# wesselb/stheno

Measured on AMD Instinct MI355X. Metric: GP logpdf+posterior evals/sec at N=16384 D=8 fp64, higher is better.
Workload: dtype f64; 1 GPU; EQ() kernel, N=16384 D=8 fp64, logpdf + condition, posterior mean/var at N*=2048; nan_scan=every step (the library's per-tensor memo is cleared at the start of each step), call_order=posterior-first, info_check=behind the call that factorised (the library's default), parallelism=replicas only (1 independent evals in flight, one process per GPU)

## Files before the change

stheno_amd/csrc/gpk_potrf.hip:

```cpp
#include "gpk_common.hpp"
#include "gpk_gemm_tile.hpp"
#include "gpk_potrf_pipe.hpp"
#include <vector>

namespace {

constexpr int LDP = 130;

template <typename T>
struct DiagArgs {
    T* A;
    int64_t ld, bstride, off;
    int n;
    T* dinv;
    int64_t dinv_bstride;
    int* info;
    int info_base;
    long long* prof;
    int zero_next;
    T* rhs = nullptr;
    int64_t rhs_stride = 0;
};

#define PROF_MARK(i)                                                            \
// ... 1074 lines not shown

void gpk_set_diag_prof(long long* dev_buf) { g_diag_prof = dev_buf; }

GPK_KNOB(int, g_batch_mixed, 1);
GPK_KNOB(int64_t, g_batch_mixed_min, 64);
GPK_KNOB(int, g_batch_lag, 96);

static bool stream_has_all_cus(hipStream_t stream) {
    if (stream == nullptr) return true;
    int dev = 0, cus = 0;
    if (hipGetDevice(&dev) != hipSuccess || hipDeviceGetAttribute(&cus, hipDeviceAttributeMultiprocessorCount, dev) != hipSuccess || cus < 1 ||
        cus > 32 * 32)
        return false;
    const uint32_t words = (uint32_t)((cus + 31) / 32);
    uint32_t mask[32];
    for (uint32_t i = 0; i < 32; ++i) mask[i] = 0u;
    if (hipExtStreamGetCUMask(stream, words, mask) != hipSuccess) {
        (void)hipGetLastError();
        return false;
    }
    int set = 0;
    for (uint32_t i = 0; i < words; ++i) set += __builtin_popcount(mask[i]);
    return set >= cus;
}

template <typename T>
struct RhsRide {
    T* B;
    int64_t sB;
    T* tmp;
    bool done;
};
template <typename T>
static int potrf_batched_mixed(T* A, int64_t n, int64_t ld, int64_t batch, int64_t bstride, T* dinv, int64_t dstride, int* info, int nbo,
                               int info_base, hipStream_t stream, RhsRide<T>* ride = nullptr) {
    const int nblk = (int)(n / GPK_DB), npb = nbo / GPK_DB;
    for (int jn = 0; jn < nblk; ++jn) {
        const bool below = jn + 1 < nblk;
        DiagArgs<T> d;
        d.A = A; d.ld = ld; d.bstride = bstride; d.off = (int64_t)jn * GPK_DB; d.n = (int)n;
        d.dinv = dinv; d.dinv_bstride = dstride; d.info = info; d.info_base = info_base;
        d.prof = g_diag_prof;
        d.zero_next = below ? 1 : 0;
        if (ride != nullptr) { d.rhs = ride->B; d.rhs_stride = ride->sB; }
        launch_diag<T>(d, (unsigned)batch, stream);
        GPK_CHECK_LAUNCH();
        if (!below) break;
        BatchStepArgs<T> p;
        p.rhs = ride != nullptr ? ride->B : nullptr;
        p.srhs = ride != nullptr ? ride->sB : 0;
        p.A = A; p.ld = ld; p.bstride = bstride; p.n = (int)n; p.batch = (int)batch;
        p.dinv = dinv; p.dstride = dstride; p.info = info;
        p.jn = jn;
        p.tm = nblk - jn - 1;
        const int jl = jn % npb;
        if (jl == npb - 1) {
            p.K = nbo; p.tn = p.tm;
        } else {
            int z = 0;
            while ((jl >> z) & 1) ++z;
            p.K = GPK_DB << z;
            p.tn = (p.K / GPK_DB < p.tm) ? p.K / GPK_DB : p.tm;
        }
        p.nU = p.tm;
        for (int ti = 1; ti < p.tm; ++ti) p.nU += (ti < p.tn - 1) ? ti : p.tn - 1;
        p.lag = (g_batch_lag + p.tm + p.nU - 1) / (p.tm + p.nU);
        const int per_xcd = (int)((batch + 7) / 8);
        if (p.lag > per_xcd) p.lag = per_xcd;
        if (p.lag < 1) p.lag = 1;
        const int64_t qlen = (int64_t)(per_xcd + p.lag) * (p.tm + p.nU);
        const int ndiag = p.tn < p.tm ? p.tn : p.tm;
        const double fl = (double)batch * ((double)p.tm * GPK_DB * GPK_DB * GPK_DB + (2.0 * (p.nU - ndiag) + ndiag) * GPK_DB * GPK_DB * (double)p.K);
        void* slot = gpk_prof_begin(160 + (sizeof(T) == 8 ? 8 : 0), fl, stream);
        hipLaunchKernelGGL((batch_mix_kernel<T>), dim3((unsigned)(8 * qlen)), dim3(256), 0, stream, p);
        gpk_prof_end(slot, stream);
        GPK_CHECK_LAUNCH();
    }
    if (ride != nullptr) ride->done = true;
    return GPK_OK;
}

template <typename T>
static int potrf_plain(T* A, int64_t n, int64_t ld, int64_t batch, int64_t bstride, T* dinv,
                       int* info, int nbo, int info_base, hipStream_t stream, int64_t rows = 0, RhsRide<T>* rhs_ride = nullptr) {
    if (n <= 0 || batch <= 0) return GPK_OK;
    if (rows < n) rows = n;
    if (rows > INT32_MAX) return GPK_ERR_ARG(2);
    if (ld < n) return GPK_ERR_ARG(3);
    if (rows > n && (batch != 1 || dinv == nullptr || !g_pipe)) return GPK_ERR_ARG(2);
    if (nbo <= 0) nbo = (batch == 1 && dinv != nullptr) ? (n <= 4096 ? 4096 : (int)g_plain_nbo) : ((n >= 8192) ? 1024 : (n >= 2048 ? 512 : 256));
    if (nbo < GPK_DB || (nbo & (nbo - 1))) return GPK_ERR_ARG(9);
    if (info == nullptr) return GPK_ERR_ARG(7);
    if (dinv == nullptr && n > GPK_DB) return GPK_ERR_ARG(6);
    const int64_t nblk = gpk_cdiv(n, GPK_DB);
    const int64_t dstride = nblk * GPK_DB * GPK_DB;

    if constexpr (sizeof(T) == 4) {
        if (g_batch_mixed && batch >= g_batch_mixed_min && rows == n && dinv != nullptr && n % GPK_DB == 0 && n >= 4 * GPK_DB && nbo <= n &&
            n <= 64 * 1024 && stream_has_all_cus(stream) && ld % Traits<T>::VEC == 0 && bstride % Traits<T>::VEC == 0 && (uintptr_t)A % 16 == 0 &&
            (uintptr_t)dinv % 16 == 0 && ld < GPK_PIPE_LD_MAX && batch <= INT32_MAX / 8)
            return potrf_batched_mixed<T>(A, n, ld, batch, bstride, dinv, dstride, info, nbo, info_base, stream, rhs_ride);
    }

    PanelCtx<T> ctx{A, n, ld, batch, bstride, dinv, dstride, info, stream, info_base};
    ctx.rows = rows;
    const bool ride = g_pipe && g_pipe_fill && batch == 1 && dinv != nullptr;
    int64_t owed = 0;
    for (int64_t k0 = 0; k0 < n; k0 += nbo) {
        const int64_t k1 = (k0 + nbo < n) ? k0 + nbo : n;
        bool done = false;
        if (owed > 0) {
            const T* P = A + k0 * ld + (k0 - owed);
            int st = gpk_gemm_launch<T>(true, true, rows - k0, k1 - k0, owed, T(-1), P, ld, bstride, P, ld, bstride, T(1), A + k0 * ld + k0, ld,
                                        bstride, batch, true, stream);
            if (st) return st;
            if (k1 < n && n - k0 > GPK_DB) {
                st = potrf_panel_pipe<T>(ctx, k0, nbo, &done, owed);
                if (st) return st;
            }
            if (!done && k1 < n) {
                const T* P2 = A + k1 * ld + (k0 - owed);
                st = gpk_gemm_launch<T>(true, true, rows - k1, n - k1, owed, T(-1), P2, ld, bstride, P2, ld, bstride, T(1), A + k1 * ld + k1, ld,
                                        bstride, batch, true, stream);
                if (st) return st;
            }
            owed = 0;
        }
        if (!done) {
            int pst = potrf_panel_any<T>(ctx, k0, nbo);
            if (pst) return pst;
        }
        if (k1 < n) {
            if (ride && n - k1 > GPK_DB) {
                owed = k1 - k0;
            } else {
                const T* P = A + k1 * ld + k0;
                int st = gpk_gemm_launch<T>(true, true, rows - k1, n - k1, k1 - k0, T(-1), P, ld, bstride, P, ld,
                                            bstride, T(1), A + k1 * ld + k1, ld, bstride, batch, true, stream);
                if (st) return st;
            }
        }
    }
    return GPK_OK;
}


#include <mutex>

namespace {

struct LaDevice {
    hipStream_t aux = nullptr;
    hipStream_t priv = nullptr;
    std::vector<hipEvent_t> events;
};
std::mutex g_la_mutex;
LaDevice g_la_dev[64];
GPK_KNOB(int64_t, g_la_min_rows, 2048);
GPK_KNOB(int64_t, g_la_tail_rows, 0);
GPK_KNOB(int, g_la_mode, 1);
GPK_KNOB(int64_t, g_la_fuse_diag_rows, 9216);
GPK_KNOB(int, g_la_fuse_diag_nb, 512);
GPK_KNOB(int, g_la_agg, 2);
GPK_KNOB(int64_t, g_la_agg_min_rows, 0);

LaDevice* la_device() {
    int dev = 0;
    if (hipGetDevice(&dev) != hipSuccess || dev < 0 || dev >= 64) return nullptr;
    LaDevice& d = g_la_dev[dev];
    if (d.aux == nullptr) {
        unsigned keys[8];
        if (gpk_helper_stream(&d.aux, keys) != GPK_OK) d.aux = nullptr;
    }
    return &d;
}

hipEvent_t la_event(LaDevice& d, size_t i) {
    while (d.events.size() <= i) {
        hipEvent_t e;
        if (hipEventCreateWithFlags(&e, hipEventDisableTiming) != hipSuccess) return nullptr;
        d.events.push_back(e);
    }
    return d.events[i];
}

template <typename T>
int la_chain(T* A, int64_t n, int64_t ld, T* dinv128, T* dinv_big, int nb, int sb, T* tmp, int* info, int64_t j,
             hipStream_t s, int max_wgs = 0, unsigned* wait_word = nullptr, unsigned wait_value = 0) {
    const int64_t k0 = j * nb;
    const int64_t w = (n - k0 < nb) ? n - k0 : nb;
// ... 21 lines not shown
        }
        for (hipEvent_t e : d.events) (void)hipEventDestroy(e);
        d = LaDevice();
    }
    (void)hipSetDevice(cur);
}

void gpk_tune_potrf(int key, int64_t value) {
    if (key == 6) GPK_KNOB_SET(g_la_min_rows = value;);
    if (key == 7) GPK_KNOB_SET(g_la_mode = (int)value;);
    if (key == 9) GPK_KNOB_SET(g_la_tail_rows = value;);
    if (key == 32) GPK_KNOB_SET(g_fused_step = (int)value;);
    if (key == 37) GPK_KNOB_SET(g_pipe = (int)value;);
    if (key == 40) GPK_KNOB_SET(g_la_fuse_diag_rows = value;);
    if (key == 41) GPK_KNOB_SET(g_la_fuse_diag_nb = (int)value;);
    if (key == 47) GPK_KNOB_SET(g_la_agg = (int)value;);
    if (key == 48) GPK_KNOB_SET(g_la_agg_min_rows = value;);
    if (key == 52) GPK_KNOB_SET(g_plain_nbo = value;);
    if (key == 53) GPK_KNOB_SET(g_batch_mixed = (int)value;);
    if (key == 54) GPK_KNOB_SET(g_batch_mixed_min = value;);
    if (key == 55) GPK_KNOB_SET(g_batch_lag = (int)value;);
    if (key == 57) GPK_KNOB_SET(g_diag_two_per_cu = (int)value;);
    if (key == 38) GPK_KNOB_SET(g_pipe_fill = (int)value;);
    if (key == 39) GPK_KNOB_SET(g_pipe_panel_wgs = (int)value;);
}

#define GPK_LA_PAD 16
int64_t gpk_potrf_la_ws_elems_impl(int64_t n, int nb) {
    return (n > nb ? n : nb) * (int64_t)(nb + GPK_LA_PAD) + (int64_t)nb * nb / 4 + 16 + 128 + nb;
}

template <typename T>
static int potrf_la_body(LaDevice* dev, T* A, int64_t n, int64_t ld, T* dinv128, T* dinv_big, int nb, int sb, T* ws, int* info,
                         hipStream_t stream, int64_t rows, int flags);

template <typename T>
int gpk_potrf_la_launch(T* A, int64_t n, int64_t ld, T* dinv128, T* dinv_big, int nb, T* ws, int* info,
                        hipStream_t stream, int sb, int64_t rows, int flags) {
    if (n <= 0) return GPK_OK;
    if (rows < n) rows = n;
    if ((flags & GPK_ROWS_RHS) && rows < n + GPK_ROWS_RHS_STRIP) return GPK_ERR_ARG(2);
    if (rows > INT32_MAX) return GPK_ERR_ARG(2);
    if (rows > n && n % GPK_DB != 0) return GPK_ERR_ARG(2);
    if (rows > n && gpk_cdiv(n, nb) > 64) return GPK_ERR_ARG(2);
    if (ld < n) return GPK_ERR_ARG(3);
    if (nb < 256 || nb > 4096 || (nb & (nb - 1))) return GPK_ERR_ARG(6);
    if (sb <= 0) sb = nb;
    if (sb < 256 || sb > nb || (sb & (sb - 1))) return GPK_ERR_ARG(10);
    if (dinv128 == nullptr || dinv_big == nullptr || ws == nullptr || info == nullptr) return GPK_ERR_ARG(4);

    std::lock_guard<std::mutex> lock(g_la_mutex);
    LaDevice* dev = la_device();
    if (dev == nullptr) return GPK_ERR_LAUNCH;
    if (stream != nullptr) return potrf_la_body<T>(dev, A, n, ld, dinv128, dinv_big, nb, sb, ws, info, stream, rows, flags);

    if (dev->priv == nullptr && hipStreamCreateWithFlags(&dev->priv, hipStreamNonBlocking) != hipSuccess) {
        dev->priv = nullptr;
        return GPK_ERR_LAUNCH;
    }
    hipEvent_t e_in = la_event(*dev, 0), e_out = la_event(*dev, 1);
    if (e_in == nullptr || e_out == nullptr) return GPK_ERR_LAUNCH;
    if (hipEventRecord(e_in, nullptr) != hipSuccess || hipStreamWaitEvent(dev->priv, e_in, 0) != hipSuccess) return GPK_ERR_LAUNCH;
    const int st = potrf_la_body<T>(dev, A, n, ld, dinv128, dinv_big, nb, sb, ws, info, dev->priv, rows, flags);
    if (hipEventRecord(e_out, dev->priv) != hipSuccess || hipStreamWaitEvent(nullptr, e_out, 0) != hipSuccess) return st ? st : GPK_ERR_LAUNCH;
    return st;
}

template <typename T>
static int potrf_la_body(LaDevice* dev, T* A, int64_t n, int64_t ld, T* dinv128, T* dinv_big, int nb, int sb, T* ws, int* info,
                         hipStream_t stream, int64_t rows, int flags) {
    const bool rhs = (flags & GPK_ROWS_RHS) != 0;
    const int64_t Rall = rows;
    const int64_t R = rhs ? rows - GPK_ROWS_RHS_STRIP : rows;
    T* bvec = rhs ? A + R * ld : nullptr;
    unsigned* const ctrl_sets[2] = {reinterpret_cast<unsigned*>(ws), reinterpret_cast<unsigned*>(ws) + GPK_PERSIST_CTRL_WORDS};
    const int64_t ldt = nb + GPK_LA_PAD;
    T* Tp = ws + 128;
    T* tmp = Tp + (Rall > nb ? Rall : nb) * ldt;
    T* vtmp = tmp + (int64_t)nb * nb / 4 + 16;
    const int64_t nblk = gpk_cdiv(n, nb);
    const int64_t per = (int64_t)sb * sb;
    size_t ev = 2;

    auto finish_plain = [&](int64_t k) -> int {
        int s = potrf_plain<T>(A + k * ld + k, n - k, ld, 1, 0, dinv128 + (k / GPK_DB) * (int64_t)(GPK_DB * GPK_DB), info,
                               0, (int)k, stream, Rall - k);
        if (s) return s;
        if (flags & GPK_ROWS_NO_TAIL_INVERSES) return GPK_OK;
        return gpk_trtri_merge_launch<T>(A + k * ld + k, n - k, ld, 1, 0, dinv128 + (k / GPK_DB) * (int64_t)(GPK_DB * GPK_DB),
                                         sb, dinv_big + (k / sb) * per, Tp, stream);
    };
    int64_t tail_rows = g_la_tail_rows > 0 ? g_la_tail_rows : 6144;
    if (Rall > n && tail_rows < nb) tail_rows = nb;
    if (n <= tail_rows) return finish_plain(0);

    hipEvent_t e_side = nullptr;
    bool side_used = false;
    hipStream_t side = nullptr;
    if (rhs && g_la_mode == 1 && dev->aux != nullptr && gpk_helper_side_stream(&side) != GPK_OK) side = nullptr;
    auto rhs_panel = [&](int64_t j) -> int {
        if (!rhs) return GPK_OK;
        hipStream_t s = stream;
        if (side != nullptr) {
            hipEvent_t e = la_event(*dev, ev++);
            if (e == nullptr || hipEventRecord(e, stream) != hipSuccess || hipStreamWaitEvent(side, e, 0) != hipSuccess) return GPK_ERR_LAUNCH;
            side_used = true;
            s = side;
        }
        const int64_t k0 = j * nb;
        for (int64_t c = 0; c < nb; c += sb) {
            const int64_t r0 = k0 + c, r1 = r0 + sb;
            const int st1 = gpk_trsv_step_launch<T>(dinv_big + (r0 / sb) * per, sb, sb, A + r1 * ld + r0, ld, n - r1, bvec + r0, bvec + r1, vtmp, s);
            if (st1) return st1;
        }
        return GPK_OK;
    };
    auto rhs_join = [&]() -> int {
        if (!side_used) return GPK_OK;
        if (e_side == nullptr) e_side = la_event(*dev, ev++);
        if (e_side == nullptr || hipEventRecord(e_side, side) != hipSuccess || hipStreamWaitEvent(stream, e_side, 0) != hipSuccess) return GPK_ERR_LAUNCH;
        return GPK_OK;
    };
    auto steps = [&]() -> int {
        int st = la_chain<T>(A, n, ld, dinv128, dinv_big, nb, sb, tmp, info, 0, stream);
        if (st) return st;
        if (nblk > 1) {
            st = gpk_copy2d_launch<T>(A + (int64_t)nb * ld, ld, 0, Tp + (int64_t)nb * ldt, ldt, 0, R - nb, nb, 1, stream);
            if (st) return st;
        }
        const int agg = (g_la_agg > 1 && nblk <= 64) ? (int)g_la_agg : 1;
        std::vector<int> applied((size_t)nblk, 0);
        struct ColGroup { int from; uint64_t mask; };
        auto group_cols = [&](int64_t c_first, int64_t j, bool all, std::vector<ColGroup>& out) {
            out.clear();
            const bool wide = nblk - c_first > 64;
            for (int64_t c = c_first; c < nblk; ++c) {
                if (!all && (c - j) % agg != 0) continue;
                size_t g = 0;
                while (g < out.size() && out[g].from != applied[(size_t)c]) ++g;
                if (g == out.size()) out.push_back(ColGroup{applied[(size_t)c], 0});
                if (wide) out[g].mask = ~(uint64_t)0;
                else out[g].mask |= (uint64_t)1 << (c - c_first);
                applied[(size_t)c] = (int)(j + 1);
            }
        };
        auto col_segment = [&](const ColGroup& cg, int64_t c_first, int64_t k1) -> GpkSeg<T> {
            const int64_t kc = c_first * nb, ka = (int64_t)cg.from * nb;
            const T* P = A + kc * ld + ka;
            const uint64_t every = (nblk - c_first >= 64) ? ~(uint64_t)0 : (((uint64_t)1 << (nblk - c_first)) - 1);
            return GpkSeg<T>{R - kc, n - kc, k1 - ka, P, ld, P, ld, A + kc * ld + kc, ld, A + kc * ld + kc, ld, 1, 0,
                             (cg.mask == every && R == n) ? 0 : cg.mask, nb};
        };
        std::vector<ColGroup> groups;
        for (int64_t j = 0; j + 1 < nblk; ++j) {
            const int64_t k0 = j * nb, k1 = k0 + nb;
            const int64_t k2 = (k1 + nb < n) ? k1 + nb : n;
            unsigned* const ctrl_step = ctrl_sets[j & 1];
            unsigned* const ctrl = ctrl_sets[(j + 1) & 1];
            if (sb < nb) {
                for (int64_t i = 0; i * sb < nb && st == GPK_OK; ++i) {
                    const int64_t c = i * sb;
                    if (i > 0)
                        st = gpk_gemm_launch<T>(true, true, R - k1, sb, c, T(-1), A + k1 * ld + k0, ld, 0, A + (k0 + c) * ld + k0, ld, 0, T(1),
                                                Tp + k1 * ldt + c, ldt, 0, 1, 0, stream);
                    if (st == GPK_OK)
                        st = gpk_gemm_launch<T>(true, true, R - k1, sb, sb, T(1), Tp + k1 * ldt + c, ldt, 0, dinv_big + (k0 / sb + i) * per, sb, 0, T(0),
                                                A + k1 * ld + k0 + c, ld, 0, 1, 8, stream);
                }
            } else {
                st = gpk_gemm_launch<T>(true, true, R - k1, nb, nb, T(1), Tp + k1 * ldt, ldt, 0, dinv_big + j * per, nb, 0, T(0),
                                        A + k1 * ld + k0, ld, 0, 1, 8, stream);
            }
            if (st) return st;
            st = rhs_panel(j);
            if (st) return st;
            if (n - k1 <= tail_rows) {
                group_cols(j + 1, j, true, groups);
                for (size_t g0 = 0; g0 < groups.size(); g0 += GPK_PERSIST_MAX_SEG) {
                    GpkSeg<T> sg[GPK_PERSIST_MAX_SEG];
                    int ns = 0;
                    for (size_t g = g0; g < groups.size() && ns < GPK_PERSIST_MAX_SEG; ++g) sg[ns++] = col_segment(groups[g], j + 1, k1);
                    st = gpk_gemm_persist_launch<T>(sg, ns, T(-1), ctrl, 0, stream);
                    if (st) return st;
                }
                st = rhs_join();
                if (st) return st;
                return finish_plain(k1);
            }
            const int64_t ka1 = (int64_t)applied[(size_t)(j + 1)] * nb, kd1 = k1 - ka1;
            applied[(size_t)(j + 1)] = (int)(j + 1);
            const T* P1 = A + k1 * ld + ka1;
            const bool overlap = g_la_mode == 1 && dev->aux != nullptr && (n - k2) >= g_la_min_rows;
            const bool fuse_diag = overlap && nb <= g_la_fuse_diag_nb && g_la_fuse_diag_rows > 0 && (n - k2) >= g_la_fuse_diag_rows && g_pipe &&
                                   (k2 - k1) > GPK_DB;
            if (!fuse_diag) {
                st = gpk_gemm_launch<T>(true, true, k2 - k1, k2 - k1, kd1, T(-1), P1, ld, 0, P1, ld, 0, T(1),
                                        A + k1 * ld + k1, ld, 0, 1, 1, stream);
                if (st) return st;
            }
            if (k2 < n) group_cols(j + 2, j, agg == 1 || (n - k2) < g_la_agg_min_rows, groups);
            else groups.clear();
            {
                const size_t room = (size_t)(GPK_PERSIST_MAX_SEG - 1 - (fuse_diag ? 1 : 0));
                while (groups.size() > room) {
                    GpkSeg<T> sg = col_segment(groups.back(), j + 2, k1);
                    groups.pop_back();
                    st = gpk_gemm_persist_launch<T>(&sg, 1, T(-1), ctrl, 0, stream);
                    if (st) return st;
                }
            }
            hipEvent_t e_fork = nullptr, e_join = nullptr;
            if (overlap) {
                e_fork = la_event(*dev, ev++);
                e_join = la_event(*dev, ev++);
                if (e_fork == nullptr || e_join == nullptr) return GPK_ERR_LAUNCH;
                if (hipMemsetAsync(ctrl_step, 0, GPK_PERSIST_CTRL_WORDS * sizeof(unsigned), stream) != hipSuccess) return GPK_ERR_LAUNCH;
                if (hipEventRecord(e_fork, stream) != hipSuccess) return GPK_ERR_LAUNCH;
            } else {
                st = la_chain<T>(A, n, ld, dinv128, dinv_big, nb, sb, tmp, info, j + 1, stream);
                if (st) return st;
            }
            GpkPersistSaved saved;
            saved.valid = 0;
            auto forked = [&]() -> int {
                if (k2 < n) {
                    const T* P2 = A + k2 * ld + ka1;
                    GpkSeg<T> seg[GPK_PERSIST_MAX_SEG];
                    int ns = 0;
                    if (fuse_diag) seg[ns++] = GpkSeg<T>{k2 - k1, k2 - k1, kd1, P1, ld, P1, ld, A + k1 * ld + k1, ld, A + k1 * ld + k1, ld, 1, 1};
                    const GpkSeg<T> strip{R - k2, k2 - k1, kd1, P2, ld, P1, ld, A + k2 * ld + k1, ld, Tp + k2 * ldt, ldt, 0};
                    for (const ColGroup& cg : groups) seg[ns++] = col_segment(cg, j + 2, k1);
                    seg[ns++] = strip;
                    const int s2 = gpk_gemm_persist_launch<T>(seg, ns, T(-1), ctrl_step, overlap ? 1 : 0, stream, &saved, overlap);
                    if (s2) return s2;
                }
                if (overlap) {
                    if (hipStreamWaitEvent(dev->aux, e_fork, 0) != hipSuccess) return GPK_ERR_LAUNCH;
                    const int s2 = fuse_diag ? la_chain<T>(A, n, ld, dinv128, dinv_big, nb, sb, tmp, info, j + 1, dev->aux, 8, ctrl_step + 2, (unsigned)saved.signal_tiles)
                                             : la_chain<T>(A, n, ld, dinv128, dinv_big, nb, sb, tmp, info, j + 1, dev->aux, 8);
                    if (s2) return s2;
                    if (saved.valid)
                        return gpk_gemm_persist_rejoin<T>(&saved, dev->aux);
                }
                return GPK_OK;
            };
            st = forked();
            if (overlap) {
                const bool joined = hipEventRecord(e_join, dev->aux) == hipSuccess && hipStreamWaitEvent(stream, e_join, 0) == hipSuccess;
                if (!joined && st == GPK_OK) st = GPK_ERR_LAUNCH;
            }
            if (st) return st;
        }
        return GPK_OK;
    };
    const int st_all = steps();
    const int st_join = rhs_join();
    return st_all ? st_all : st_join;
}

template int gpk_potrf_la_launch<double>(double*, int64_t, int64_t, double*, double*, int, double*, int*, hipStream_t, int, int64_t, int);
template int gpk_potrf_la_launch<float>(float*, int64_t, int64_t, float*, float*, int, float*, int*, hipStream_t, int, int64_t, int);

template <typename T>
int gpk_potrf_launch(T* A, int64_t n, int64_t ld, int64_t batch, int64_t bstride, T* dinv,
                     int* info, int nbo, hipStream_t stream) {
    return potrf_plain<T>(A, n, ld, batch, bstride, dinv, info, nbo, 0, stream);
}

template <typename T>
int gpk_potrf_rhs_launch(T* A, int64_t n, int64_t ld, int64_t batch, int64_t bstride, T* dinv, int* info, int nbo, T* B, int64_t sB, T* tmp,
                         hipStream_t stream) {
    if (B == nullptr || tmp == nullptr || dinv == nullptr) return GPK_ERR_ARG(9);
    if (batch > 1 && sB < n) return GPK_ERR_ARG(10);
    RhsRide<T> ride{B, sB, tmp, false};
    int st = potrf_plain<T>(A, n, ld, batch, bstride, dinv, info, nbo, 0, stream, 0, &ride);
    if (st) return st;
    if (!ride.done) st = gpk_trsv_launch<T>(A, n, ld, bstride, dinv, GPK_DB, B, 1, 1, sB, tmp, batch, stream);
    return st;
}
template int gpk_potrf_rhs_launch<double>(double*, int64_t, int64_t, int64_t, int64_t, double*, int*, int, double*, int64_t, double*, hipStream_t);
template int gpk_potrf_rhs_launch<float>(float*, int64_t, int64_t, int64_t, int64_t, float*, int*, int, float*, int64_t, float*, hipStream_t);

template <typename T>
int gpk_potrf_rows_launch(T* A, int64_t n, int64_t rows, int64_t ld, T* dinv, int* info, hipStream_t stream) {
    return potrf_plain<T>(A, n, ld, 1, 0, dinv, info, 0, 0, stream, rows);
}
template int gpk_potrf_rows_launch<double>(double*, int64_t, int64_t, int64_t, double*, int*, hipStream_t);
template int gpk_potrf_rows_launch<float>(float*, int64_t, int64_t, int64_t, float*, int*, hipStream_t);

template int gpk_potrf_launch<double>(double*, int64_t, int64_t, int64_t, int64_t, double*, int*,
                                      int, hipStream_t);
template int gpk_potrf_launch<float>(float*, int64_t, int64_t, int64_t, int64_t, float*, int*, int,
                                     hipStream_t);
```

stheno_amd/csrc/selftest.cpp:

```cpp
#include <hip/hip_runtime.h>
#include <algorithm>
#include <chrono>
#include <cmath>
#include <cstdio>
#include <cstdlib>
#include <climits>
#include <cstring>
#include <random>
#include <string>
#include <limits>
#include <vector>
#include <atomic>
#include <functional>
#include <thread>
#include "../../include/gpk.h"

#define HIPCHK(x)                                                                       \
    do {                                                                                \
        hipError_t e = (x);                                                             \
        if (e != hipSuccess) {                                                          \
            printf("HIP error %s at %s:%d\n", hipGetErrorString(e), __FILE__, __LINE__); \
            exit(3);                                                                    \
        }                                                                               \
    } while (0)
// ... 652 lines not shown
            zn = std::max(zn, std::fabs(g - z[j])); zd = std::max(zd, std::fabs(z[j]));
        }
        znum_e[e] = zn; zden_e[e] = zd; bad_e[e] = bad;
    });
    for (int e = 0; e < extra; ++e) {
        if (bad_e[e]) finite = false;
        znum = std::max(znum, znum_e[e]); zden = std::max(zden, zden_e[e]);
    }
    char nm[200];
    snprintf(nm, sizeof nm, "potrf_rows_%s n%d +%d rows nb%d sb%d tail%lld agg%d flags%d st%d/%d info%d: factor", DT<T>::name(), n, extra, nb, wb, (long long)tail, agg, flags, st, st2, info.down()[0]);
    report(nm, (st || st2 || !finite || info.down()[0]) ? INFINITY : num / den, DT<T>::eps);
    snprintf(nm, sizeof nm, "potrf_rows_%s n%d +%d rows nb%d sb%d tail%lld agg%d flags%d: rows = E L^-T", DT<T>::name(), n, extra, nb, wb, (long long)tail, agg, flags);
    report(nm, (st || !finite) ? INFINITY : znum / zden, DT<T>::eps * 2);
}

template <typename T>
static void test_potrf_rhs_case(int n, int batch) {
    const int64_t ld = n, bs = (int64_t)n * ld;
    auto A = make_spd<T>(n, batch, ld);
    auto Bv = randv<T>((size_t)batch * n);
    Dev<T> dA(A.size()), dR(A.size()), dinv((size_t)batch * gpk_dinv_elems(n)), dinv2((size_t)batch * gpk_dinv_elems(n)), dB(Bv.size()), dB2(Bv.size()),
        tmp((size_t)batch * 128 + 16), tmp2((size_t)batch * 128 + 16);
    Dev<int> info(batch), info2(batch);
    dA.up(A); dR.up(A); dB.up(Bv); dB2.up(Bv); info.zero(); info2.zero();
    const int st = gpk_potrf_rhs(DT<T>::v, dA.p, n, ld, bs, batch, dinv.p, info.p, 0, dB.p, n, tmp.p, nullptr);
    const int st2 = gpk_potrf(DT<T>::v, dR.p, n, ld, bs, batch, dinv2.p, info2.p, 0, nullptr);
    const int st3 = gpk_trsv_lower(DT<T>::v, dR.p, n, ld, bs, dinv2.p, 128, dB2.p, 1, 1, n, tmp2.p, batch, nullptr);
    HIPCHK(hipDeviceSynchronize());
    auto G = dA.down(), R = dR.down();
    auto x = dB.down(), x2 = dB2.down();
    size_t diff = 0;
    for (int b = 0; b < batch; ++b)
        for (int i = 0; i < n; ++i)
            for (int j = 0; j <= i; ++j) diff += G[(size_t)b * bs + (size_t)i * ld + j] != R[(size_t)b * bs + (size_t)i * ld + j];
    double num = 0, den = 0;
    bool finite = true;
    for (size_t i = 0; i < x.size(); ++i) {
        if (!std::isfinite((double)x[i])) finite = false;
        num = std::max(num, std::fabs((double)x[i] - (double)x2[i])); den = std::max(den, std::fabs((double)x2[i]));
    }
    int bad = 0;
    for (int v : info.down()) bad += v != 0;
    char nm[200];
    snprintf(nm, sizeof nm, "potrf_rhs_%s n%d batch%d st%d/%d/%d bad_info%d: factors differ in %zu entries", DT<T>::name(), n, batch, st, st2, st3, bad, diff);
    report(nm, (st || st2 || st3 || bad || diff) ? INFINITY : 0.0, DT<T>::eps);
    snprintf(nm, sizeof nm, "potrf_rhs_%s n%d batch%d: L^-1 b against gpk_trsv_lower", DT<T>::name(), n, batch);
    report(nm, (st || !finite) ? INFINITY : num / den, DT<T>::eps * 200);
}

template <typename T>
static void test_potrf_rhs() {
    test_potrf_rhs_case<T>(512, 64);
    test_potrf_rhs_case<T>(1024, 70);
    test_potrf_rhs_case<T>(2048, 64);
    test_potrf_rhs_case<T>(640, 9);
    test_potrf_rhs_case<T>(300, 5);
    test_potrf_rhs_case<T>(1024, 1);
}

template <typename T>
static void test_potrf_rows() {
    test_potrf_rows_case<T>(128, 64, 0, 0, 0);
    test_potrf_rows_case<T>(640, 200, 0, 0, 0);
    test_potrf_rows_case<T>(1024, 300, 0, 0, 0);
    test_potrf_rows_case<T>(2560, 333, 0, 0, 0);
    test_potrf_rows_case<T>(5120, 260, 0, 0, 0);
    test_potrf_rows_case<T>(3072, 300, 512, 0, 1024);
    test_potrf_rows_case<T>(3072, 300, 512, 256, 1024);
    test_potrf_rows_case<T>(4096, 520, 1024, 0, 2048, 1);
    test_potrf_rows_case<T>(4096, 130, 256, 0, 512, 3);
    test_potrf_rows_case<T>(3840, 1000, 256, 0, 100, 2);
    test_potrf_rows_case<T>(2048, 77, 256, 0, 0);
    test_potrf_rows_case<T>(2176, 130, 0, 0, 0);
    test_potrf_rows_case<T>(4224, 64, 0, 0, 0);
    test_potrf_rows_case<T>(5248, 200, 0, 0, 0);
    test_potrf_rows_case<T>(4224, 96, 1024, 0, 2048);
    test_potrf_rows_case<T>(7296, 64, 1024, 512, 3072);
    test_potrf_rows_case<T>(640, 65, 0, 0, 0, 2, 1);
    test_potrf_rows_case<T>(3072, 301, 512, 0, 1024, 2, 1);
    test_potrf_rows_case<T>(3072, 65, 512, 256, 1024, 2, 3);
    test_potrf_rows_case<T>(4096, 1, 1024, 0, 2048, 1, 1);
    test_potrf_rows_case<T>(7296, 129, 1024, 512, 3072, 2, 3);
    test_potrf_rows_case<T>(2048, 78, 256, 0, 0, 2, 3);
}

template <typename T>
static void test_lookahead() {
    for (int pass = 0; pass < 2; ++pass) {
        gpk_tune(1, pass == 0 ? 0 : ((int64_t)1 << 40));
        test_update2_case<T>(300, 200, 260, 70, 0, 0);
        test_update2_case<T>(384, 128, 512, 64, 1, 0);
        test_update2_case<T>(1000, 256, 1100, 128, 1, 2);
        test_update2_case<T>(129, 1, 5, 3, 1, 1);
    }
    gpk_tune(1, 512);
    test_potrf_la_case<T>(700, 256, 1, 0);
    test_potrf_la_case<T>(1024, 256, 1, 0);
    test_potrf_la_case<T>(1200, 512, 1, 0);
    test_potrf_la_case<T>(1664, 256, 0, 0);
    test_potrf_la_case<T>(3000, 512, 1, 0);
    test_potrf_la_case<T>(3000, 1024, 1, 1024);
    test_potrf_la_case<T>(4096, 1024, 1, 0);
    test_potrf_la_case<T>(5000, 512, 1, 2048);
    test_potrf_la_case<T>(4096, 1024, 1, 0, 0, 512);
    test_potrf_la_case<T>(5000, 1024, 1, 1024, 1000, 256);
    test_potrf_la_case<T>(3000, 512, 1, 0, 700, 256);
    test_potrf_la_case<T>(2100, 1024, 0, 0, 300, 512);
    gpk_tune(40, 256); gpk_tune(41, 4096);
    test_potrf_la_case<T>(4096, 1024, 1, 0);
    test_potrf_la_case<T>(5000, 512, 1, 1024);
    test_potrf_la_case<T>(6000, 256, 1, 0, 700);
    gpk_tune(40, 9216); gpk_tune(41, 512);
    test_potrf_la_case<T>(10, 256, 1, 0, 5120);
    test_potrf_la_case<T>(1200, 512, 1, 0, 5120);
    test_potrf_la_case<T>(1664, 256, 1, 0, 700);
    test_potrf_la_case<T>(3000, 512, 1, 0, 1500);
    test_potrf_la_case<T>(4096, 1024, 1, 0, 2048);
    test_potrf_la_case<T>(5000, 1024, 1, 1024, 1000);
    for (int m : {1, 2, 3, 4, 7}) {
        gpk_tune(47, m);
        test_potrf_la_case<T>(3000, 256, 1, 0, 300);
        test_potrf_la_case<T>(4100, 512, 1, 1024, 600);
        test_potrf_la_case<T>(2900, 256, 0, 0, 300, 128 * 2);
        gpk_tune(48, 1800);
        test_potrf_la_case<T>(3333, 256, 1, 0, 500);
        gpk_tune(48, 0);
        gpk_tune(40, 256); gpk_tune(41, 4096);
        test_potrf_la_case<T>(3000, 256, 1, 0, 300);
        gpk_tune(48, 1500);
        test_potrf_la_case<T>(3000, 256, 1, 0, 300);
        gpk_tune(48, 0);
        gpk_tune(40, 9216); gpk_tune(41, 512);
    }
    gpk_tune(47, 2);
    test_potrf_la_case<T>(16896, 256, 1, 0, 1024);
    {
        const int n = 1500, nb = 512, bad = 1111;
        const int64_t ld = n;
        auto A = make_spd<T>(n, 1, ld);
        A[(size_t)bad * ld + bad] = (T)(-5);
        Dev<T> dA(A.size()), dinv((size_t)gpk_dinv_elems(n)), dbig((size_t)3 * nb * nb), ws((size_t)gpk_potrf_la_ws_elems(n, nb));
        Dev<int> info(1);
        dA.up(A); info.zero();
        for (int64_t tail : {0, 700}) {
            dA.up(A); info.zero();
            gpk_tune(6, 0); gpk_tune(9, tail);
            const int st = gpk_potrf_la(DT<T>::v, dA.p, n, ld, dinv.p, dbig.p, nb, ws.p, info.p, nullptr);
            gpk_tune(6, 2048); gpk_tune(9, 0);
            HIPCHK(hipDeviceSynchronize());
            char nm[160];
            snprintf(nm, sizeof nm, "potrf_la_%s not PD (tail %lld): info %d (expect %d) st%d", DT<T>::name(), (long long)tail, info.down()[0], bad + 1, st);
            report(nm, (st == 0 && info.down()[0] == bad + 1) ? 0.0 : INFINITY, 0.0);
        }
    }
}

__global__ void census_kernel(unsigned* out) {
    unsigned xcc, hw;
    asm volatile("s_getreg_b32 %0, hwreg(HW_REG_XCC_ID)" : "=s"(xcc));
    asm volatile("s_getreg_b32 %0, hwreg(HW_REG_HW_ID)" : "=s"(hw));
    if (threadIdx.x == 0) { out[2 * blockIdx.x] = xcc; out[2 * blockIdx.x + 1] = hw; }
    const long long t0 = wall_clock64();
    while (wall_clock64() - t0 < 2000) {}
}
static void census() {
    const int nb = 2048;
// ... 1634 lines not shown
        if (!strcmp(argv[i], "--cumask")) { cumask_experiment(); return 0; }
        if (!strcmp(argv[i], "--dispatch")) { dispatch_experiment(); return 0; }
        if (!strcmp(argv[i], "--tileprof")) {
            const int k = (i + 1 < argc && atoi(argv[i + 1]) > 0) ? atoi(argv[i + 1]) : 1024;
            tile_profile(k, (i + 2 < argc) ? atoi(argv[i + 2]) : 1, (i + 3 < argc) ? atoi(argv[i + 3]) : 0);
            return 0;
        }
        if (!strcmp(argv[i], "--mfmapeak")) { mfma_peak(); return 0; }
        if (!strcmp(argv[i], "--diagprof") && i + 1 < argc) {
            rsq_precision();
            for (int ver = 0; ver < 3; ++ver) {
                diag_phase_profile<double>(atoi(argv[i + 1]), ver > 0, ver == 2);
                diag_phase_profile<float>(atoi(argv[i + 1]), ver > 0, ver == 2);
            }
            return 0;
        }
        if (!strcmp(argv[i], "--profile") && i + 3 < argc) {
            const int n = atoi(argv[i + 2]), nbo = atoi(argv[i + 3]);
            if (!strcmp(argv[i + 1], "f64")) profile_one<double>(n, nbo, 2); else profile_one<float>(n, nbo, 2);
            return 0;
        }
        if (!strcmp(argv[i], "--gemm") && i + 4 < argc) {
            const int M = atoi(argv[i + 2]), N = atoi(argv[i + 3]), K = atoi(argv[i + 4]);
            const int flags = (i + 5 < argc) ? atoi(argv[i + 5]) : 0;
            const int64_t lda = (i + 6 < argc) ? atoll(argv[i + 6]) : -1;
            if (!strcmp(argv[i + 1], "f64")) gemm_one<double>(M, N, K, flags, 4, lda); else gemm_one<float>(M, N, K, flags, 4, lda);
            return 0;
        }
        if (!strcmp(argv[i], "--census")) { census(); return 0; }
        if (!strcmp(argv[i], "--perf-kmat")) { perf_kmat(); return 0; }
        if (!strcmp(argv[i], "--perf-diff")) {
            for (int lower = 1; lower >= 0; --lower) { perf_diff_case<double>(16384, 8, lower); perf_diff_case<float>(16384, 8, lower); }
            return 0;
        }
        if (!strcmp(argv[i], "--perf-fill") && i + 1 < argc) {
            const int n = atoi(argv[i + 1]);
            for (int wg : {-1, 16, 32, 48, 64, 85, 128, 170}) {
                gpk_tune(38, wg < 0 ? 0 : 1);
                gpk_tune(39, wg < 0 ? 0 : wg);
                printf("FILL panel workgroups %d (fill %s):\n", wg, wg < 0 ? "off" : "on");
                perf_la_tail<double>({n});
                perf_la_tail<float>({n});
            }
            gpk_tune(38, 1); gpk_tune(39, 0);
            return 0;
        }
        if (!strcmp(argv[i], "--perf-la-tail")) { perf_la_tail<double>({6144, 8192, 10240, 12288, 16384}); perf_la_tail<float>({8192, 12288, 16384, 32768}); return 0; }
        if (!strcmp(argv[i], "--perf-pipe")) { perf_pipe<double>(); perf_pipe<float>(); return 0; }
        if (!strcmp(argv[i], "--perf-trsv")) { perf_trsv<double>(16384, {512, 1024, 2048}); perf_trsv<float>(32768, {256, 512, 1024}); return 0; }
        if (!strcmp(argv[i], "--perf-trsm")) { perf_trsm<double>(16384, 2048); perf_trsm<float>(32768, 2048); return 0; }
        if (!strcmp(argv[i], "--kmat")) {
            for (int band = 1; band >= 0; --band) { gpk_tune(12, band); test_kmat<double>(); test_kmat<float>(); }
            printf("SUMMARY pass=%d fail=%d\n", g_pass, g_fail);
            return g_fail ? 1 : 0;
        }
        if (!strcmp(argv[i], "--rq")) {
            test_rq<double>(); test_rq<float>();
            printf("SUMMARY pass=%d fail=%d\n", g_pass, g_fail);
            return g_fail ? 1 : 0;
        }
        if (!strcmp(argv[i], "--diff")) {
            test_diff<double>(); test_diff<float>();
            printf("SUMMARY pass=%d fail=%d\n", g_pass, g_fail);
            return g_fail ? 1 : 0;
        }
        if (!strcmp(argv[i], "--delta")) {
            test_delta<double>(); test_delta<float>();
            printf("SUMMARY pass=%d fail=%d\n", g_pass, g_fail);
            return g_fail ? 1 : 0;
        }
        if (!strcmp(argv[i], "--potrf")) {
            test_potrf<double>(); test_potrf<float>();
            test_lookahead<double>(); test_lookahead<float>();
            printf("SUMMARY pass=%d fail=%d\n", g_pass, g_fail);
            return g_fail ? 1 : 0;
        }
        if (!strcmp(argv[i], "--rows")) {
            test_potrf_rows<double>(); test_potrf_rows<float>();
        test_potrf_rhs<double>(); test_potrf_rhs<float>();
            test_potrf_rhs<double>(); test_potrf_rhs<float>();
            printf("SUMMARY pass=%d fail=%d\n", g_pass, g_fail);
            return g_fail ? 1 : 0;
        }
        if (!strcmp(argv[i], "--lookahead")) {
            test_lookahead<double>(); test_lookahead<float>();
            printf("SUMMARY pass=%d fail=%d\n", g_pass, g_fail);
            return g_fail ? 1 : 0;
        }
        if (!strcmp(argv[i], "--la-one") && i + 5 < argc) {
            const int n = atoi(argv[i + 2]), nb = atoi(argv[i + 3]), mode = atoi(argv[i + 4]);
            const int64_t mr = atoll(argv[i + 5]);
            const int reps = (i + 6 < argc) ? atoi(argv[i + 6]) : 3;
            const int ldpad = (i + 7 < argc) ? atoi(argv[i + 7]) : 0;
            if (!strcmp(argv[i + 1], "f64")) la_one<double>(n, nb, mode, mr, reps, ldpad); else la_one<float>(n, nb, mode, mr, reps, ldpad);
            return 0;
        }
        if (!strcmp(argv[i], "--perf-agg") && i + 6 < argc) {
            const int n = atoi(argv[i + 2]), nb = atoi(argv[i + 3]), sb = atoi(argv[i + 4]), rounds = atoi(argv[i + 5]);
            const int64_t tail = atoll(argv[i + 6]);
            std::vector<int> ml;
            for (int q = i + 7; q < argc && argv[q][0] != '-'; ++q) ml.push_back(atoi(argv[q]));
            if (ml.empty()) ml = {1, 2};
            if (!strcmp(argv[i + 1], "f64")) perf_agg<double>(n, nb, sb, rounds, ml, tail); else perf_agg<float>(n, nb, sb, rounds, ml, tail);
            return 0;
        }
        if (!strcmp(argv[i], "--perf-rows") && i + 6 < argc) {
            const int n = atoi(argv[i + 2]), extra = atoi(argv[i + 3]), nb = atoi(argv[i + 4]), sb = atoi(argv[i + 5]), rounds = atoi(argv[i + 6]);
            if (!strcmp(argv[i + 1], "f64")) perf_rows<double>(n, extra, nb, sb, rounds); else perf_rows<float>(n, extra, nb, sb, rounds);
            return 0;
        }
        if (!strcmp(argv[i], "--la-clock") && i + 3 < argc) {
            const int warm = (i + 4 < argc) ? atoi(argv[i + 4]) : 0;
            if (!strcmp(argv[i + 1], "f64")) la_clock<double>(atoi(argv[i + 2]), atoi(argv[i + 3]), warm); else la_clock<float>(atoi(argv[i + 2]), atoi(argv[i + 3]), warm);
            return 0;
        }
        if (!strcmp(argv[i], "--perf-la")) {
            const int nmax = (i + 1 < argc && atoi(argv[i + 1]) > 0) ? atoi(argv[i + 1]) : 16384;
            perf_la<double>(nmax); perf_la<float>(nmax);
            return 0;
        }
        if (!strcmp(argv[i], "--perf")) do_perf = true;
        if (!strcmp(argv[i], "--only-perf")) do_perf = only_perf = true;
    }
    hipDeviceProp_t prop;
    HIPCHK(hipGetDeviceProperties(&prop, 0));
    printf("device: %s  arch=%s  CUs=%d  clock=%d MHz  gpk_version=%d\n", prop.name, prop.gcnArchName, prop.multiProcessorCount, prop.clockRate / 1000, gpk_version());
    if (!only_perf) {
        test_probe<double>(); test_probe<float>();
        gpk_tune(1, 0);
        test_gemm<double>(); test_gemm<float>();
        gpk_tune(1, (int64_t)1 << 40);
        test_gemm<double>(); test_gemm<float>();
        gpk_tune(1, 512);
        test_kmat<double>(); test_kmat<float>();
        test_potrf<double>(); test_potrf<float>();
        test_lookahead<double>(); test_lookahead<float>();
        test_potrf_rows<double>(); test_potrf_rows<float>();
        test_potrf_rhs<double>(); test_potrf_rhs<float>();
        test_misc<double>(); test_misc<float>();
        test_vjp_dense<double>(); test_vjp_dense<float>();
        test_rq<double>(); test_rq<float>();
        test_delta<double>(); test_delta<float>();
        test_diff<double>(); test_diff<float>();
        printf("SUMMARY pass=%d fail=%d\n", g_pass, g_fail);
    }
    if (do_perf) { perf<double>(); perf<float>(); }
    return g_fail ? 1 : 0;
}
```

Before: 29.08 evals/s.

## Hand over from lookahead Cholesky to plain tail one step early with owed update

The lookahead Cholesky now detects the step before the tail and hands over to the plain panel factorisation one block early. The trailing update of the last lookahead panel is passed in as an 'owed' update instead of being applied separately. The default tail threshold drops from 6144 to 5120 rows, while the whole-matrix plain path keeps the old 6144 cutoff. The aim is to avoid a separate trailing-update launch and a serial step at the boundary, at the cost of more complex hand-over logic, including RHS solves limited to the rows above the tail.

```diff
diff --git a/stheno_amd/csrc/gpk_potrf.hip b/stheno_amd/csrc/gpk_potrf.hip
--- a/stheno_amd/csrc/gpk_potrf.hip
+++ b/stheno_amd/csrc/gpk_potrf.hip
@@ -1180,8 +1180,9 @@
 
 template <typename T>
 static int potrf_plain(T* A, int64_t n, int64_t ld, int64_t batch, int64_t bstride, T* dinv,
-                       int* info, int nbo, int info_base, hipStream_t stream, int64_t rows = 0, RhsRide<T>* rhs_ride = nullptr) {
+                       int* info, int nbo, int info_base, hipStream_t stream, int64_t rows = 0, RhsRide<T>* rhs_ride = nullptr, int64_t owed_in = 0) {
     if (n <= 0 || batch <= 0) return GPK_OK;
+    if (owed_in < 0 || (owed_in > 0 && batch != 1)) return GPK_ERR_ARG(2);
     if (rows < n) rows = n;
     if (rows > INT32_MAX) return GPK_ERR_ARG(2);
     if (ld < n) return GPK_ERR_ARG(3);
@@ -1203,7 +1204,7 @@
     PanelCtx<T> ctx{A, n, ld, batch, bstride, dinv, dstride, info, stream, info_base};
     ctx.rows = rows;
     const bool ride = g_pipe && g_pipe_fill && batch == 1 && dinv != nullptr;
-    int64_t owed = 0;
+    int64_t owed = owed_in;
     for (int64_t k0 = 0; k0 < n; k0 += nbo) {
         const int64_t k1 = (k0 + nbo < n) ? k0 + nbo : n;
         bool done = false;
@@ -1391,23 +1392,23 @@
     const int64_t per = (int64_t)sb * sb;
     size_t ev = 2;
 
-    auto finish_plain = [&](int64_t k) -> int {
+    auto finish_plain = [&](int64_t k, int64_t owed = 0) -> int {
         int s = potrf_plain<T>(A + k * ld + k, n - k, ld, 1, 0, dinv128 + (k / GPK_DB) * (int64_t)(GPK_DB * GPK_DB), info,
-                               0, (int)k, stream, Rall - k);
+                               0, (int)k, stream, Rall - k, nullptr, owed);
         if (s) return s;
         if (flags & GPK_ROWS_NO_TAIL_INVERSES) return GPK_OK;
         return gpk_trtri_merge_launch<T>(A + k * ld + k, n - k, ld, 1, 0, dinv128 + (k / GPK_DB) * (int64_t)(GPK_DB * GPK_DB),
                                          sb, dinv_big + (k / sb) * per, Tp, stream);
     };
-    int64_t tail_rows = g_la_tail_rows > 0 ? g_la_tail_rows : 6144;
+    int64_t tail_rows = g_la_tail_rows > 0 ? g_la_tail_rows : 5120;
     if (Rall > n && tail_rows < nb) tail_rows = nb;
-    if (n <= tail_rows) return finish_plain(0);
+    if (n <= (g_la_tail_rows > 0 ? tail_rows : 6144)) return finish_plain(0);
 
     hipEvent_t e_side = nullptr;
     bool side_used = false;
     hipStream_t side = nullptr;
     if (rhs && g_la_mode == 1 && dev->aux != nullptr && gpk_helper_side_stream(&side) != GPK_OK) side = nullptr;
-    auto rhs_panel = [&](int64_t j) -> int {
+    auto rhs_panel = [&](int64_t j, int64_t below) -> int {
         if (!rhs) return GPK_OK;
         hipStream_t s = stream;
         if (side != nullptr) {
@@ -1419,7 +1420,7 @@
         const int64_t k0 = j * nb;
         for (int64_t c = 0; c < nb; c += sb) {
             const int64_t r0 = k0 + c, r1 = r0 + sb;
-            const int st1 = gpk_trsv_step_launch<T>(dinv_big + (r0 / sb) * per, sb, sb, A + r1 * ld + r0, ld, n - r1, bvec + r0, bvec + r1, vtmp, s);
+            const int st1 = gpk_trsv_step_launch<T>(dinv_big + (r0 / sb) * per, sb, sb, A + r1 * ld + r0, ld, below - r1, bvec + r0, bvec + r1, vtmp, s);
             if (st1) return st1;
         }
         return GPK_OK;
@@ -1460,12 +1461,9 @@
             return GpkSeg<T>{R - kc, n - kc, k1 - ka, P, ld, P, ld, A + kc * ld + kc, ld, A + kc * ld + kc, ld, 1, 0,
                              (cg.mask == every && R == n) ? 0 : cg.mask, nb};
         };
-        std::vector<ColGroup> groups;
-        for (int64_t j = 0; j + 1 < nblk; ++j) {
+        auto solve = [&](int64_t j) -> int {
             const int64_t k0 = j * nb, k1 = k0 + nb;
-            const int64_t k2 = (k1 + nb < n) ? k1 + nb : n;
-            unsigned* const ctrl_step = ctrl_sets[j & 1];
-            unsigned* const ctrl = ctrl_sets[(j + 1) & 1];
+            int st = GPK_OK;
             if (sb < nb) {
                 for (int64_t i = 0; i * sb < nb && st == GPK_OK; ++i) {
                     const int64_t c = i * sb;
@@ -1480,10 +1478,20 @@
                 st = gpk_gemm_launch<T>(true, true, R - k1, nb, nb, T(1), Tp + k1 * ldt, ldt, 0, dinv_big + j * per, nb, 0, T(0),
                                         A + k1 * ld + k0, ld, 0, 1, 8, stream);
             }
+            return st;
+        };
+        std::vector<ColGroup> groups;
+        for (int64_t j = 0; j + 1 < nblk; ++j) {
+            const int64_t k0 = j * nb, k1 = k0 + nb;
+            const int64_t k2 = (k1 + nb < n) ? k1 + nb : n;
+            unsigned* const ctrl_step = ctrl_sets[j & 1];
+            unsigned* const ctrl = ctrl_sets[(j + 1) & 1];
+            st = solve(j);
             if (st) return st;
-            st = rhs_panel(j);
+            st = rhs_panel(j, n);
             if (st) return st;
-            if (n - k1 <= tail_rows) {
+            const bool to_tail = k2 < n && n - k2 <= tail_rows;
+            if (!to_tail && n - k1 <= tail_rows) {
                 group_cols(j + 1, j, true, groups);
                 for (size_t g0 = 0; g0 < groups.size(); g0 += GPK_PERSIST_MAX_SEG) {
                     GpkSeg<T> sg[GPK_PERSIST_MAX_SEG];
@@ -1507,7 +1515,7 @@
                                         A + k1 * ld + k1, ld, 0, 1, 1, stream);
                 if (st) return st;
             }
-            if (k2 < n) group_cols(j + 2, j, agg == 1 || (n - k2) < g_la_agg_min_rows, groups);
+            if (k2 < n) group_cols(j + 2, j, to_tail || agg == 1 || (n - k2) < g_la_agg_min_rows, groups);
             else groups.clear();
             {
                 const size_t room = (size_t)(GPK_PERSIST_MAX_SEG - 1 - (fuse_diag ? 1 : 0));
@@ -1559,6 +1567,15 @@
                 if (!joined && st == GPK_OK) st = GPK_ERR_LAUNCH;
             }
             if (st) return st;
+            if (to_tail) {
+                st = solve(j + 1);
+                if (st) return st;
+                st = rhs_panel(j + 1, k2);
+                if (st) return st;
+                st = rhs_join();
+                if (st) return st;
+                return finish_plain(k2, k2 - k1);
+            }
         }
         return GPK_OK;
     };
diff --git a/stheno_amd/csrc/selftest.cpp b/stheno_amd/csrc/selftest.cpp
--- a/stheno_amd/csrc/selftest.cpp
+++ b/stheno_amd/csrc/selftest.cpp
@@ -758,6 +758,45 @@
     test_potrf_rows_case<T>(4096, 1, 1024, 0, 2048, 1, 1);
     test_potrf_rows_case<T>(7296, 129, 1024, 512, 3072, 2, 3);
     test_potrf_rows_case<T>(2048, 78, 256, 0, 0, 2, 3);
+}
+
+template <typename T>
+static void test_tail_entry() {
+    for (int n : {1536, 1280, 1664}) {
+        test_potrf_la_case<T>(n, 256, 1, 256, 512);
+        gpk_tune(6, 256);
+        test_potrf_rows_case<T>(n, 128, 256, 0, 512);
+        test_potrf_rows_case<T>(n, 129, 256, 0, 512, 2, 1);
+        gpk_tune(6, 2048);
+    }
+    test_potrf_la_case<T>(1280, 256, 1, 256, 256);
+    gpk_tune(6, 256);
+    test_potrf_rows_case<T>(1280, 128, 256, 0, 256);
+    test_potrf_rows_case<T>(1280, 129, 256, 0, 256, 2, 3);
+    test_potrf_rows_case<T>(1536, 129, 512, 256, 512, 2, 1);
+    test_potrf_rows_case<T>(1536, 129, 256, 0, 512, 1, 1);
+    test_potrf_rows_case<T>(7168, 64, 1024, 0, 0, 2, 1);
+    gpk_tune(6, 2048);
+    {
+        const int n = 1536, nb = 256, bad = 900, extra = 128;
+        const int64_t ld = n, rows = n + extra + GPK_ROWS_RHS_STRIP;
+        auto A = make_spd<T>(n, 1, ld);
+        A[(size_t)bad * ld + bad] = (T)(-5);
+        std::vector<T> full((size_t)rows * ld, T(0));
+        std::copy(A.begin(), A.end(), full.begin());
+        auto E = randv<T>((size_t)(extra + 1) * ld);
+        std::copy(E.begin(), E.end(), full.begin() + (size_t)n * ld);
+        Dev<T> dA(full.size()), dinv((size_t)gpk_dinv_elems(n) + 128 * 128), dbig((size_t)(n / nb) * nb * nb), ws((size_t)gpk_potrf_la_ws_elems(rows, nb));
+        Dev<int> info(1);
+        dA.up(full); info.zero();
+        gpk_tune(6, 256); gpk_tune(9, 512);
+        const int st = gpk_potrf_rows_rhs(DT<T>::v, dA.p, n, rows, ld, dinv.p, dbig.p, nb, 0, ws.p, info.p, GPK_ROWS_RHS, nullptr);
+        gpk_tune(6, 2048); gpk_tune(9, 0);
+        const bool synced = hipDeviceSynchronize() == hipSuccess;
+        char nm[200];
+        snprintf(nm, sizeof nm, "potrf_rows_%s not PD in the hand-over step's chain: info %d (expect %d) st%d synced%d", DT<T>::name(), info.down()[0], bad + 1, st, (int)synced);
+        report(nm, (st == 0 && synced && info.down()[0] == bad + 1) ? 0.0 : INFINITY, 0.0);
+    }
 }
 
 template <typename T>
@@ -2558,6 +2597,11 @@
             printf("SUMMARY pass=%d fail=%d\n", g_pass, g_fail);
             return g_fail ? 1 : 0;
         }
+        if (!strcmp(argv[i], "--tail-entry")) {
+            test_tail_entry<double>(); test_tail_entry<float>();
+            printf("SUMMARY pass=%d fail=%d\n", g_pass, g_fail);
+            return g_fail ? 1 : 0;
+        }
         if (!strcmp(argv[i], "--lookahead")) {
             test_lookahead<double>(); test_lookahead<float>();
             printf("SUMMARY pass=%d fail=%d\n", g_pass, g_fail);
@@ -2612,6 +2656,7 @@
         test_potrf<double>(); test_potrf<float>();
         test_lookahead<double>(); test_lookahead<float>();
         test_potrf_rows<double>(); test_potrf_rows<float>();
+        test_tail_entry<double>(); test_tail_entry<float>();
         test_potrf_rhs<double>(); test_potrf_rhs<float>();
         test_misc<double>(); test_misc<float>();
         test_vjp_dense<double>(); test_vjp_dense<float>();
```

Result: faster. 29.40 evals/s (median of 6 runs) (+1.1%).
